# andrewjong/SwapNet

Hardware: NVIDIA H100
Metric: images/sec (G+D fwd+bwd) warp-stage 512x512 (higher is better)
Workload: dtype fp16/bf16-split x3 tensor-core products, fp32 accumulate (fp32-faithful)

## Files before the change

### swapnet_b200/csrc/common.cuh

```cuda
#pragma once
#include <cuda_runtime.h>
#include <cuda.h>
#include <cuda_bf16.h>
#include <cuda_fp16.h>
#include <stdint.h>
#include <stdio.h>
#include <string.h>

void sn_set_error(const char* fmt, ...);
#define SN_OK 0
#define SN_ERR_INVALID (-1)
#define SN_ERR_CUDA (-2)
#define SN_ERR_UNSUPPORTED (-3)
#define SN_NUM_SMS 132
#ifndef SN_FMT_BF16
#define SN_FMT_BF16 0
#define SN_FMT_F16 1
#endif

#define SN_CHECK_CUDA(expr)                                                        \
  do {                                                                             \
    cudaError_t _e = (expr);                                                       \
    if (_e != cudaSuccess) {                                                       \
      sn_set_error("%s:%d CUDA error %s: %s", __FILE__, __LINE__, #expr,           \
                   cudaGetErrorString(_e));                                        \
      return SN_ERR_CUDA;                                                          \
    }                                                                              \
  } while (0)

#define SN_REQUIRE(cond, ...)                                                      \
  do {                                                                             \
    if (!(cond)) {                                                                 \
      sn_set_error(__VA_ARGS__);                                                   \
      return SN_ERR_INVALID;                                                       \
    }                                                                              \
  } while (0)

#ifdef __CUDACC__

__device__ __forceinline__ uint32_t smem_u32(const void* p) {
  return static_cast<uint32_t>(__cvta_generic_to_shared(p));
}

__device__ __forceinline__ bool elect_one_sync() {
  uint32_t pred = 0;
  asm volatile(
      "{\n\t"
      ".reg .pred P;\n\t"
      "elect.sync _|P, 0xffffffff;\n\t"
      "selp.b32 %0, 1, 0, P;\n\t"
      "}\n"
      : "=r"(pred));
  return pred != 0;
}

__device__ __forceinline__ void mbar_init(uint64_t* bar, uint32_t count) {
  asm volatile("mbarrier.init.shared::cta.b64 [%0], %1;" ::"r"(smem_u32(bar)), "r"(count));
}
__device__ __forceinline__ void mbar_fence_init() {
  asm volatile("fence.mbarrier_init.release.cluster;" ::: "memory");
}
__device__ __forceinline__ void mbar_expect_tx(uint64_t* bar, uint32_t bytes) {
  asm volatile("mbarrier.arrive.expect_tx.shared::cta.b64 _, [%0], %1;" ::"r"(smem_u32(bar)),
               "r"(bytes)
               : "memory");
}
__device__ __forceinline__ void mbar_arrive(uint64_t* bar) {
  asm volatile("mbarrier.arrive.shared::cta.b64 _, [%0];" ::"r"(smem_u32(bar)) : "memory");
}
__device__ __forceinline__ bool mbar_try_wait(uint64_t* bar, uint32_t parity) {
  uint32_t ok;
  asm volatile(
      "{\n\t"
      ".reg .pred P;\n\t"
      "mbarrier.try_wait.parity.shared::cta.b64 P, [%1], %2;\n\t"
      "selp.b32 %0, 1, 0, P;\n\t"
      "}\n"
      : "=r"(ok)
      : "r"(smem_u32(bar)), "r"(parity)
      : "memory");
  return ok != 0;
}
__device__ __forceinline__ void mbar_wait(uint64_t* bar, uint32_t parity) {
  uint32_t spins = 0;
  while (!mbar_try_wait(bar, parity)) {
    if (++spins > (1u << 28)) __trap();
  }
}

__device__ __forceinline__ void tma_prefetch_desc(const void* desc) {
  asm volatile("prefetch.tensormap [%0];" ::"l"(reinterpret_cast<uint64_t>(desc)) : "memory");
}
__device__ __forceinline__ void tma_load_2d(const void* desc, uint64_t* bar, void* dst, int c0,
                                            int c1) {
  asm volatile(
      "cp.async.bulk.tensor.2d.shared::cluster.global.mbarrier::complete_tx::bytes"
      " [%0], [%1, {%3, %4}], [%2];"
      :
      : "r"(smem_u32(dst)), "l"(reinterpret_cast<uint64_t>(desc)), "r"(smem_u32(bar)), "r"(c0),
        "r"(c1)
      : "memory");
}
__device__ __forceinline__ void tma_load_3d(const void* desc, uint64_t* bar, void* dst, int c0, int c1, int c2) {
  asm volatile(
      "cp.async.bulk.tensor.3d.shared::cluster.global.mbarrier::complete_tx::bytes"
      " [%0], [%1, {%3, %4, %5}], [%2];"
      :
      : "r"(smem_u32(dst)), "l"(reinterpret_cast<uint64_t>(desc)), "r"(smem_u32(bar)), "r"(c0), "r"(c1), "r"(c2)
      : "memory");
}
__device__ __forceinline__ void tma_load_5d(const void* desc, uint64_t* bar, void* dst, int c0,
                                            int c1, int c2, int c3, int c4) {
  asm volatile(
      "cp.async.bulk.tensor.5d.shared::cluster.global.mbarrier::complete_tx::bytes"
      " [%0], [%1, {%3, %4, %5, %6, %7}], [%2];"
      :
      : "r"(smem_u32(dst)), "l"(reinterpret_cast<uint64_t>(desc)), "r"(smem_u32(bar)), "r"(c0),
        "r"(c1), "r"(c2), "r"(c3), "r"(c4)
      : "memory");
}

__device__ __forceinline__ void wgmma_fence() { asm volatile("wgmma.fence.sync.aligned;" ::: "memory"); }
__device__ __forceinline__ void wgmma_commit() { asm volatile("wgmma.commit_group.sync.aligned;" ::: "memory"); }
template <int N>
__device__ __forceinline__ void wgmma_wait() {
  asm volatile("wgmma.wait_group.sync.aligned %0;" ::"n"(N) : "memory");
}
template <int R>
__device__ __forceinline__ void wgmma_fence_acc(float (&d)[R]) {
#pragma unroll
  for (int i = 0; i < R; ++i) asm volatile("" : "+f"(d[i])::"memory");
}

template <int N, bool F16>
struct Wgmma;
template <> struct Wgmma<16, false> {
  template <int TA, int TB>
  static __device__ __forceinline__ void mma(float (&d)[8], uint64_t a, uint64_t b, int scale_d) {
    asm volatile(
        "{\n.reg .pred p;\nsetp.ne.b32 p, %10, 0;\n"
        "wgmma.mma_async.sync.aligned.m64n16k16.f32.bf16.bf16 "
        "{%0, %1, %2, %3, %4, %5, %6, %7}, %8, %9, p, 1, 1, %11, %12;\n}\n"
        : "+f"(d[0]), "+f"(d[1]), "+f"(d[2]), "+f"(d[3]), "+f"(d[4]), "+f"(d[5]), "+f"(d[6]), "+f"(d[7])
        : "l"(a), "l"(b), "r"(scale_d), "n"(TA), "n"(TB));
  }
};
template <> struct Wgmma<16, true> {
  template <int TA, int TB>
  static __device__ __forceinline__ void mma(float (&d)[8], uint64_t a, uint64_t b, int scale_d) {
    asm volatile(
        "{\n.reg .pred p;\nsetp.ne.b32 p, %10, 0;\n"
        "wgmma.mma_async.sync.aligned.m64n16k16.f32.f16.f16 "
        "{%0, %1, %2, %3, %4, %5, %6, %7}, %8, %9, p, 1, 1, %11, %12;\n}\n"
        : "+f"(d[0]), "+f"(d[1]), "+f"(d[2]), "+f"(d[3]), "+f"(d[4]), "+f"(d[5]), "+f"(d[6]), "+f"(d[7])
        : "l"(a), "l"(b), "r"(scale_d), "n"(TA), "n"(TB));
  }
};
template <> struct Wgmma<32, false> {
// ... 145 lines not shown
```

### swapnet_b200/csrc/gemm_tc.cu

```cuda
#include "common.cuh"
#include "plan.h"

namespace {

constexpr int kBlockM = 128;
constexpr int kTileRing = 4;
constexpr int kTileBytes = 16384;
constexpr int kConsumerWarps = 8;
constexpr int kProducerWarp = kConsumerWarps;
constexpr int kThreads = (kConsumerWarps + 1) * 32;

template <int NSPLIT>
struct Cfg {
  static constexpr int kPlanes = NSPLIT == 3 ? 2 : 1;
  static constexpr int kStages = NSPLIT == 3 ? 3 : 6;
  static constexpr int kStageBytes = kPlanes * 2 * kTileBytes;
  static constexpr int kSmemBytes = kStages * kStageBytes + 1024;
};

__device__ __forceinline__ float apply_act(float v, int act) {
  if (act == SN_ACT_TANH) return tanhf(v);
  return v;
}

__device__ __forceinline__ float quad_col_sum(float v) {
  v += __shfl_xor_sync(0xffffffffu, v, 4);
  v += __shfl_xor_sync(0xffffffffu, v, 8);
  v += __shfl_xor_sync(0xffffffffu, v, 16);
  return v;
}

template <int NSPLIT, int CW, int BN, bool F16>
__global__ void __launch_bounds__(kThreads, 1)
tap_gemm_kernel(const __grid_constant__ TapGemmParams p, const int m_tiles, const int n_tiles, const int total_tiles) {
  const auto tile_coords = [&](int tile, int& mt, int& nt, int& z) {
    nt = tile % n_tiles;
    const int rest = tile / n_tiles;
    mt = rest % m_tiles;
    z = rest / m_tiles;
  };
  using C = Cfg<NSPLIT>;
  extern __shared__ uint8_t smem_raw[];
  __shared__ __align__(8) uint64_t full_bar[C::kStages];
  __shared__ __align__(8) uint64_t empty_bar[C::kStages];
  __shared__ __align__(8) uint64_t tr_full[kTileRing];
  __shared__ __align__(8) uint64_t tr_empty[kTileRing];
  __shared__ int tile_ring[kTileRing];

  const uint32_t smem_base = (smem_u32(smem_raw) + 1023u) & ~1023u;
  uint8_t* smem = smem_raw + (smem_base - smem_u32(smem_raw));
  const int warp = threadIdx.x >> 5;
  const int lane = threadIdx.x & 31;

  constexpr int cw = CW;
  constexpr int tps = 64 / cw;
  const int tpp = p.ntaps / p.nphase;
  const int k_iters = cw == 64 ? tpp * p.chunks : tpp / tps;

  if (threadIdx.x == 0) {
    for (int s = 0; s < C::kStages; ++s) {
      mbar_init(&full_bar[s], 1);
      mbar_init(&empty_bar[s], 2);
    }
    for (int r = 0; r < kTileRing; ++r) {
      mbar_init(&tr_full[r], 1);
      mbar_init(&tr_empty[r], kConsumerWarps);
    }
    mbar_fence_init();
  }
  if (warp == kProducerWarp && lane == 0) {
    for (int pl = 0; pl < C::kPlanes; ++pl) {
      tma_prefetch_desc(&p.tmA[pl]);
      tma_prefetch_desc(&p.tmB[pl]);
    }
  }
  __syncthreads();

  if (warp == kProducerWarp) {
    if (lane == 0) {
      const uint32_t stage_tx = C::kPlanes * (p.a_rows * 128 + p.block_n * 128);
      uint32_t it = 0, tcount = 0;
      for (int tile = blockIdx.x;; ++tcount) {
        const int next = tile < total_tiles ? (int)gridDim.x + atomicAdd(p.tile_counter, 1) : total_tiles;
        const uint32_t slot = tcount % kTileRing, rph = (tcount / kTileRing) & 1;
        mbar_wait(&tr_empty[slot], rph ^ 1);
        tile_ring[slot] = tile < total_tiles ? tile : -1;
        mbar_arrive(&tr_full[slot]);
        if (tile >= total_tiles) break;
        int mt, nt, z;
        tile_coords(tile, mt, nt, z);
        const int ncol0 = nt * p.block_n;
        const int tap0 = z * tpp;
        const int w0 = (mt % p.tiles_w) * p.tw;
// ... 116 lines not shown
        optr[h] = p.out + (long long)gn[h] * p.out_sn + (long long)(gh[h] * p.omh + p.ooh + ph_h) * p.out_sh +
                  (long long)(gw[h] * p.omw + p.oow + ph_w) * p.out_sw + ncol0;
      }
#pragma unroll
      for (int i = 0; i < BN / 8; ++i) {
        const int c = 8 * i + 2 * quad;
        if (BN > 16 && 8 * i >= p.block_n) break;
        if (p.stack_slot) {
#pragma unroll
          for (int h = 0; h < 2; ++h) {
            if (!valid[h]) continue;
#pragma unroll
            for (int e = 0; e < 2; ++e) {
              const int col = ncol0 + c + e;
              const int ph = col / p.stack_slot, ch = col - ph * p.stack_slot;
              if (ph < 4 && ch < p.stack_c) {
                float v = acc[4 * i + 2 * h + e] * oscale;
                if (p.bias) v += p.bias[ch];
                float* o = p.out + (long long)gn[h] * p.out_sn + (long long)(gh[h] * p.omh + (ph >> 1)) * p.out_sh +
                           (long long)(gw[h] * p.omw + (ph & 1)) * p.out_sw + ch;
                *o = apply_act(v, p.act);
              }
            }
          }
        } else if (p.stats) {
          if (ncol0 + 8 * i >= p.n_valid) continue;
          float v[2][2];
#pragma unroll
          for (int h = 0; h < 2; ++h) {
#pragma unroll
            for (int e = 0; e < 2; ++e) {
              float t = acc[4 * i + 2 * h + e] * oscale;
              if (p.bias) t += p.bias[ncol0 + c + e];
              v[h][e] = valid[h] ? t : 0.f;
            }
            if (valid[h]) *reinterpret_cast<float2*>(optr[h] + c) = make_float2(v[h][0], v[h][1]);
          }
          const float s0 = quad_col_sum(v[0][0] + v[1][0]);
          const float s1 = quad_col_sum(v[0][1] + v[1][1]);
          const float q0 = quad_col_sum(v[0][0] * v[0][0] + v[1][0] * v[1][0]);
          const float q1 = quad_col_sum(v[0][1] * v[0][1] + v[1][1] * v[1][1]);
          if (lane < 4) {
            const int tn = (mt / (p.tiles_w * p.tiles_h)) * p.nb;
            double* sp = p.stats + ((long long)tn * p.n_valid + ncol0 + c) * 2;
            atomicAdd(sp, (double)s0);
            atomicAdd(sp + 1, (double)q0);
            atomicAdd(sp + 2, (double)s1);
            atomicAdd(sp + 3, (double)q1);
          }
        } else {
#pragma unroll
          for (int h = 0; h < 2; ++h) {
            if (!valid[h]) continue;
            float v0 = acc[4 * i + 2 * h] * oscale, v1 = acc[4 * i + 2 * h + 1] * oscale;
            const int col = ncol0 + c;
            if (p.vec4 && col + 1 < p.n_valid) {
              if (p.bias) {
                const float2 bb = *reinterpret_cast<const float2*>(p.bias + col);
                v0 += bb.x; v1 += bb.y;
              }
              *reinterpret_cast<float2*>(optr[h] + c) = make_float2(apply_act(v0, p.act), apply_act(v1, p.act));
            } else {
              if (col < p.n_valid) optr[h][c] = apply_act(p.bias ? v0 + p.bias[col] : v0, p.act);
              if (col + 1 < p.n_valid) optr[h][c + 1] = apply_act(p.bias ? v1 + p.bias[col + 1] : v1, p.act);
            }
          }
        }
      }
    }
  }

  __syncthreads();
  if (threadIdx.x == 0) {
    __threadfence();
    if (atomicAdd(p.tile_counter + 1, 1) == (int)gridDim.x - 1) {
      p.tile_counter[0] = 0;
      p.tile_counter[1] = 0;
      __threadfence();
    }
  }
}

template <int NSPLIT, int BN, bool F16, bool DET>
__global__ void __launch_bounds__(kThreads, 1)
wgrad_gemm_kernel(const __grid_constant__ WgradParams p) {
  using C = Cfg<NSPLIT>;
  extern __shared__ uint8_t smem_raw[];
  __shared__ __align__(8) uint64_t full_bar[C::kStages];
  __shared__ __align__(8) uint64_t empty_bar[C::kStages];

  const uint32_t smem_base = (smem_u32(smem_raw) + 1023u) & ~1023u;
  uint8_t* smem = smem_raw + (smem_base - smem_u32(smem_raw));
  const int warp = threadIdx.x >> 5;
  const int lane = threadIdx.x & 31;

  const int m_tile = blockIdx.x / p.n_tiles;
  const int n_tile = blockIdx.x - m_tile * p.n_tiles;
  const bool grouped = p.ngroups > 0;
  const int tap_i = grouped ? p.gstart[blockIdx.y] : blockIdx.y;
  const int gsize = grouped ? p.gsize[blockIdx.y] : 1;
  const int m0 = m_tile * kBlockM;
  const int ncol0 = n_tile * p.block_n;
  const int total = p.tiles_w * p.tiles_h * p.tiles_n;
  const int kt0 = (int)(((long long)total * blockIdx.z) / gridDim.z);
  const int kt1 = (int)(((long long)total * (blockIdx.z + 1)) / gridDim.z);
  const int k_iters = kt1 - kt0;
  const int ycw = p.y_chunk;
  const int y_blocks = ycw == 64 ? p.block_n / 64 : gsize;
  const int y_block_bytes = 64 * ycw * 2;

  if (threadIdx.x == 0) {
    for (int s = 0; s < C::kStages; ++s) {
      mbar_init(&full_bar[s], 1);
      mbar_init(&empty_bar[s], 2);
    }
    mbar_fence_init();
  }
  if (warp == kProducerWarp && lane == 0) {
    for (int pl = 0; pl < C::kPlanes; ++pl) {
      tma_prefetch_desc(&p.tmX[pl]);
      tma_prefetch_desc(&p.tmY[pl]);
    }
  }
  __syncthreads();

  if (k_iters > 0) {
    if (warp == kProducerWarp) {
      if (lane == 0) {
        const TapDesc xt = p.xtaps[tap_i];
        const uint32_t stage_tx = C::kPlanes * (2 * 8192 + y_blocks * y_block_bytes);
        for (int it = 0; it < k_iters; ++it) {
          const int s = it % C::kStages;
          const uint32_t ph = (it / C::kStages) & 1;
          mbar_wait(&empty_bar[s], ph ^ 1);
          mbar_expect_tx(&full_bar[s], stage_tx);
          const int kt = kt0 + it;
          const int tw_i = kt % p.tiles_w;
          const int th_i = (kt / p.tiles_w) % p.tiles_h;
          const int tn_i = kt / (p.tiles_w * p.tiles_h);
          const int w0 = tw_i * p.tw, h0 = th_i * p.th, n0 = tn_i * p.nb;
          uint8_t* st = smem + s * C::kStageBytes;
          if (p.x_merged) {
            for (int b = 0; b < 2; ++b)
              tma_load_5d(&p.tmX[0], &full_bar[s], st + b * 16384, xt.c_off + m0 + b * 64, w0 + xt.dw, h0 + xt.dh,
                          n0, 0);
          } else {
#pragma unroll
            for (int pl = 0; pl < C::kPlanes; ++pl)
              for (int b = 0; b < 2; ++b)
                tma_load_5d(&p.tmX[pl], &full_bar[s], st + pl * kTileBytes + b * 8192,
                            xt.c_off + m0 + b * 64, w0 + xt.dw, xt.hp, h0 + xt.dh, n0);
          }
          if (p.y_merged) {
            const TapDesc yt = p.ytaps[tap_i];
            for (int b = 0; b < y_blocks; ++b)
              tma_load_5d(&p.tmY[0], &full_bar[s], st + C::kPlanes * kTileBytes + b * 16384,
                          yt.c_off + ncol0 + b * 64, w0 + yt.dw, h0 + yt.dh, n0, 0);
          } else {
#pragma unroll
            for (int pl = 0; pl < C::kPlanes; ++pl)
              for (int b = 0; b < y_blocks; ++b) {
                const TapDesc yt = p.ytaps[grouped ? tap_i + b : tap_i];
                tma_load_5d(&p.tmY[pl], &full_bar[s],
                            st + (C::kPlanes + pl) * kTileBytes + b * y_block_bytes,
                            yt.c_off + (grouped ? 0 : ncol0 + b * 64), w0 + yt.dw, yt.hp, h0 + yt.dh, n0);
              }
          }
        }
      }
    } else if (warp < kProducerWarp) {
      const int wg = warp >> 2;
      float acc[BN / 2], part[BN / 2];
#pragma unroll
      for (int i = 0; i < BN / 2; ++i) acc[i] = 0.f;
      const uint32_t y_layout = gmma_layout_of_chunk(ycw);
      const uint32_t y_sbo = 8u * ycw * 2u;
      const uint32_t x_lbo = p.x_merged ? 16384u : 8192u;
      const uint32_t x_lo_off = p.x_merged ? 8192u : (uint32_t)kTileBytes;
      const uint32_t y_lbo = p.y_merged ? 16384u : (uint32_t)y_block_bytes;
      const uint32_t y_lo_off = p.y_merged ? 8192u : (uint32_t)kTileBytes;
      for (int it = 0; it < k_iters; ++it) {
        const int s = it % C::kStages;
        const uint32_t ph = (it / C::kStages) & 1;
        mbar_wait(&full_bar[s], ph);
        const uint32_t st = smem_base + s * C::kStageBytes;
        const uint64_t x_hi = gmma_smem_desc(st + wg * x_lbo, x_lbo, 1024);
        const uint64_t y_hi = gmma_smem_desc(st + C::kPlanes * kTileBytes, y_lbo, y_sbo, y_layout);
        const uint64_t x_lo = gmma_smem_desc(st + x_lo_off + wg * x_lbo, x_lbo, 1024);
        const uint64_t y_lo = gmma_smem_desc(st + C::kPlanes * kTileBytes + y_lo_off, y_lbo, y_sbo, y_layout);
        wgmma_fence();
#pragma unroll
        for (int k = 0; k < 4; ++k) {
          const uint64_t xadv = (uint64_t)(k * 128);
          const uint64_t yadv = (uint64_t)((k * 16 * ycw * 2) >> 4);
          Wgmma<BN, F16>::template mma<1, 1>(part, x_hi + xadv, y_hi + yadv, k != 0);
          if (NSPLIT == 3) {
            Wgmma<BN, F16>::template mma<1, 1>(part, x_lo + xadv, y_hi + yadv, 1);
            Wgmma<BN, F16>::template mma<1, 1>(part, x_hi + xadv, y_lo + yadv, 1);
          }
        }
        wgmma_commit();
        wgmma_wait<0>();
        wgmma_fence_acc(part);
        if ((threadIdx.x & 127) == 0) mbar_arrive(&empty_bar[s]);
#pragma unroll
        for (int i = 0; i < BN / 2; ++i) acc[i] += part[i];
      }
      const int quad = lane & 3;
      const int row0 = m0 + wg * 64 + (warp & 3) * 16 + (lane >> 2);
#pragma unroll
      for (int h = 0; h < 2; ++h) {
        const int row = row0 + 8 * h;
        if (row >= p.rows_valid) continue;
        float* orow = p.out + (long long)row * p.s_row;
        float* wrow = DET ? p.det_ws + (long long)blockIdx.z * p.det_count + (long long)row * p.cols_valid : nullptr;
#pragma unroll
        for (int i = 0; i < BN / 8; ++i) {
#pragma unroll
          for (int e = 0; e < 2; ++e) {
            const int c = 8 * i + 2 * quad + e;
            const float v = acc[4 * i + 2 * h + e];
            if (!grouped) {
              const int col = ncol0 + c;
              if (c < p.block_n && col < p.cols_valid) {
                if constexpr (DET) wrow[(long long)tap_i * p.rows_valid * p.cols_valid + col] = v;
                else atomicAdd(orow + p.tap_off[tap_i] + (long long)col * p.s_col, v);
              }
            } else {
              const int b = c / ycw;
              const int cbase = c - b * ycw;
              if (b < gsize && cbase < p.cols_valid) {
                if constexpr (DET) wrow[(long long)(tap_i + b) * p.rows_valid * p.cols_valid + cbase] = v;
                else atomicAdd(orow + p.tap_off[tap_i + b] + (long long)cbase * p.s_col, v);
              }
            }
          }
        }
      }
    }
  }
}

__global__ void __launch_bounds__(256) wgrad_det_sum_kernel(const __grid_constant__ WgradParams p, int ksplit) {
  const long long rc = (long long)p.rows_valid * p.cols_valid;
  for (long long e = blockIdx.x * (long long)blockDim.x + threadIdx.x; e < p.det_count;
       e += (long long)gridDim.x * blockDim.x) {
    float s = p.det_ws[e];
    for (int z = 1; z < ksplit; ++z) s += p.det_ws[(long long)z * p.det_count + e];
    const int tap = (int)(e / rc);
    const long long r = e - tap * rc;
    const int row = (int)(r / p.cols_valid), col = (int)(r - (long long)row * p.cols_valid);
    p.out[(long long)row * p.s_row + p.tap_off[tap] + (long long)col * p.s_col] += s;
  }
}

}

void sn_count_launch(int n);
typedef CUresult (*PFN_encodeTiled)(CUtensorMap*, CUtensorMapDataType, cuuint32_t, void*,
                                    const cuuint64_t*, const cuuint64_t*, const cuuint32_t*,
                                    const cuuint32_t*, CUtensorMapInterleave, CUtensorMapSwizzle,
                                    CUtensorMapL2promotion, CUtensorMapFloatOOBfill);

static PFN_encodeTiled get_encode_fn() {
  static PFN_encodeTiled fn = nullptr;
  if (!fn) {
    void* ptr = nullptr;
    cudaDriverEntryPointQueryResult qres;
    cudaError_t e = cudaGetDriverEntryPoint("cuTensorMapEncodeTiled", &ptr, cudaEnableDefault, &qres);
    if (e != cudaSuccess || qres != cudaDriverEntryPointSuccess || !ptr) return nullptr;
    fn = reinterpret_cast<PFN_encodeTiled>(ptr);
  }
  return fn;
}

int sn_make_act_map(CUtensorMap* tm, const void* base, int N, int H, int W, int C, int pitch,
                    int parity, int box_w, int box_h, int box_n, int chunk = 64, long long plane_stride = 0) {
  PFN_encodeTiled enc = get_encode_fn();
  SN_REQUIRE(enc != nullptr, "cuTensorMapEncodeTiled driver entry point unavailable");
  SN_REQUIRE(pitch % 8 == 0 && ((uintptr_t)base % 16) == 0,
             "activation plane needs 16-B aligned base and pitch %% 8 == 0 (pitch=%d)", pitch);
  SN_REQUIRE(box_w >= 1 && box_h >= 1 && box_n >= 1 && box_w <= 256 && box_h <= 256 && box_n <= 256,
             "bad TMA box %d x %d x %d", box_w, box_h, box_n);
  cuuint64_t dims[5];
  cuuint64_t strides[4];
  const cuuint64_t e = 2;
  cuuint32_t box[5] = {(cuuint32_t)chunk, (cuuint32_t)box_w, 1, (cuuint32_t)box_h, (cuuint32_t)box_n};
  if (plane_stride > 0) {
    SN_REQUIRE(plane_stride % 16 == 0, "merged planes: 16-B aligned plane stride");
    if (!parity) {
      dims[0] = C; dims[1] = W; dims[2] = H; dims[3] = N; dims[4] = 2;
      strides[0] = (cuuint64_t)pitch * e;
      strides[1] = (cuuint64_t)W * pitch * e;
    } else {
      SN_REQUIRE(H % 2 == 0 && W % 2 == 0, "parity view needs even H, W (got %d x %d)", H, W);
      dims[0] = (cuuint64_t)(W + 1) * pitch + C; dims[1] = W / 2; dims[2] = H / 2; dims[3] = N; dims[4] = 2;
      strides[0] = (cuuint64_t)2 * pitch * e;
      strides[1] = (cuuint64_t)2 * W * pitch * e;
    }
    strides[2] = (cuuint64_t)H * W * pitch * e;
    strides[3] = (cuuint64_t)plane_stride;
    box[2] = (cuuint32_t)box_h; box[3] = (cuuint32_t)box_n; box[4] = 2;
  } else if (!parity) {
    dims[0] = C; dims[1] = W; dims[2] = 1; dims[3] = H; dims[4] = N;
    strides[0] = (cuuint64_t)pitch * e;
    strides[1] = (cuuint64_t)W * pitch * e;
    strides[2] = (cuuint64_t)W * pitch * e;
    strides[3] = (cuuint64_t)H * W * pitch * e;
  } else {
    SN_REQUIRE(H % 2 == 0 && W % 2 == 0, "parity view needs even H, W (got %d x %d)", H, W);
    dims[0] = (cuuint64_t)pitch + C; dims[1] = W / 2; dims[2] = 2; dims[3] = H / 2; dims[4] = N;
    strides[0] = (cuuint64_t)2 * pitch * e;
    strides[1] = (cuuint64_t)W * pitch * e;
    strides[2] = (cuuint64_t)2 * W * pitch * e;
    strides[3] = (cuuint64_t)H * W * pitch * e;
  }
  SN_REQUIRE(chunk == 64 || chunk == 32 || chunk == 16, "row chunk must be 64, 32 or 16 channels (got %d)", chunk);
  cuuint32_t estr[5] = {1, 1, 1, 1, 1};
// ... 277 lines not shown
  for (int t = 0; t < d->ntaps; ++t) {
    p.xtaps[t].c_off = d->xtaps[t].c_off; p.xtaps[t].dw = (short)d->xtaps[t].dw;
    p.xtaps[t].dh = (short)d->xtaps[t].dh; p.xtaps[t].hp = (short)d->xtaps[t].hp;
    p.ytaps[t].c_off = d->ytaps[t].c_off; p.ytaps[t].dw = (short)d->ytaps[t].dw;
    p.ytaps[t].dh = (short)d->ytaps[t].dh; p.ytaps[t].hp = (short)d->ytaps[t].hp;
    p.tap_off[t] = d->tap_off[t];
  }
  p.block_n = d->block_n;
  p.m_tiles = (d->rows_valid + kBlockM - 1) / kBlockM;
  p.n_tiles = y_chunk == 64 ? (d->cols_valid + d->block_n - 1) / d->block_n : 1;
  p.rows_valid = d->rows_valid;
  p.cols_valid = d->cols_valid;
  p.out = d->out;
  p.s_row = d->s_row;
  p.s_col = d->s_col;
  p.x_fmt = d->x_fmt;
  p.y_fmt = d->y_fmt;
  int rc;
  const void* x_pl[2] = {d->x_hi, d->x_lo};
  const void* y_pl[2] = {d->y_hi, d->y_lo};
  {
    const long long x_ps = d->nsplit == 3 ? (const char*)d->x_lo - (const char*)d->x_hi : 0;
    const long long y_ps = d->nsplit == 3 ? (const char*)d->y_lo - (const char*)d->y_hi : 0;
    p.x_merged = x_ps > 0 && x_ps % 16 == 0 && tw * th * nb == 64;
    p.y_merged = y_ps > 0 && y_ps % 16 == 0 && tw * th * nb == 64 && y_chunk == 64 && d->ngroups == 0;
    for (int t = 0; t < d->ntaps; ++t) {
      if (p.x_merged && d->x_parity) p.xtaps[t].c_off += p.xtaps[t].hp * d->x_w * d->x_pitch;
      if (p.y_merged && d->y_parity) p.ytaps[t].c_off += p.ytaps[t].hp * d->y_w * d->y_pitch;
    }
    for (int pl = 0; pl < (d->nsplit == 3 ? 2 : 1); ++pl) {
      if (!(p.x_merged && pl == 1)) {
        rc = sn_make_act_map(&p.tmX[pl], x_pl[pl], d->x_n, d->x_h, d->x_w, d->x_c, d->x_pitch,
                             d->x_parity, tw, th, nb, 64, p.x_merged ? x_ps : 0);
        if (rc) return rc;
      }
      if (!(p.y_merged && pl == 1)) {
        rc = sn_make_act_map(&p.tmY[pl], y_pl[pl], d->y_n, d->y_h, d->y_w, d->y_c, d->y_pitch,
                             d->y_parity, tw, th, nb, y_chunk, p.y_merged ? y_ps : 0);
        if (rc) return rc;
      }
    }
    if (p.x_merged) p.tmX[1] = p.tmX[0];
    if (p.y_merged) p.tmY[1] = p.tmY[0];
  }
  plan->nsplit = d->nsplit;
  const int base_ctas = p.m_tiles * p.n_tiles * grid_y;
  const int total = p.tiles_w * p.tiles_h * p.tiles_n;
  const int ks = wgrad_ksplit(d, base_ctas, total, sm_count);
  plan->grid = dim3(p.m_tiles * p.n_tiles, grid_y, ks);
  p.det_ws = nullptr;
  p.det_count = 0;
  plan->ws_bytes = 0;
  if (d->deterministic) {
    for (int t = 0; t < d->ntaps; ++t)
      for (int u = 0; u < t; ++u)
        SN_REQUIRE(d->tap_off[t] != d->tap_off[u], "deterministic wgrad: taps %d and %d share tap_off", u, t);
    p.det_count = (long long)d->ntaps * d->rows_valid * d->cols_valid;
    plan->ws_bytes = sizeof(float) * (size_t)ks * p.det_count;
    SN_CHECK_CUDA(cudaMalloc(&p.det_ws, plan->ws_bytes));
  }
  return SN_OK;
}

int sn_wgrad_plan_ksplit(const sn_wgrad_desc* d, int sm_count) {
  SN_REQUIRE(d && d->ntaps >= 1 && d->ntaps <= SN_MAX_TAPS, "wgrad_ksplit: bad descriptor");
  int th, tw, nb;
  pick_patch(d->m_h, d->m_w, 64, &th, &tw, &nb);
  const int total = ((d->m_w + tw - 1) / tw) * ((d->m_h + th - 1) / th) * ((d->m_n + nb - 1) / nb);
  const int y_chunk = d->y_chunk ? d->y_chunk : 64;
  const int grid_y = (y_chunk != 64 && d->ngroups > 0) ? d->ngroups : d->ntaps;
  const int m_tiles = (d->rows_valid + kBlockM - 1) / kBlockM;
  const int n_tiles = y_chunk == 64 ? (d->cols_valid + d->block_n - 1) / d->block_n : 1;
  return wgrad_ksplit(d, m_tiles * n_tiles * grid_y, total, sm_count);
}

template <int NSPLIT, int BN, bool F16, bool DET>
static int launch_wgrad_k(const WgradPlan* plan, cudaStream_t stream) {
  static bool attr_done = false;
  if (!attr_done) {
    SN_CHECK_CUDA(cudaFuncSetAttribute(wgrad_gemm_kernel<NSPLIT, BN, F16, DET>,
                                       cudaFuncAttributeMaxDynamicSharedMemorySize, Cfg<NSPLIT>::kSmemBytes));
    attr_done = true;
  }
  wgrad_gemm_kernel<NSPLIT, BN, F16, DET><<<plan->grid, kThreads, Cfg<NSPLIT>::kSmemBytes, stream>>>(plan->p);
  SN_CHECK_CUDA(cudaGetLastError());
  return SN_OK;
}

template <int NSPLIT, int BN, bool F16>
static int launch_wgrad(const WgradPlan* plan, cudaStream_t stream) {
  if (!plan->p.det_ws) return launch_wgrad_k<NSPLIT, BN, F16, false>(plan, stream);
  const int rc = launch_wgrad_k<NSPLIT, BN, F16, true>(plan, stream);
  if (rc) return rc;
  long long g = (plan->p.det_count + 255) / 256;
  if (g > SN_NUM_SMS * 8) g = SN_NUM_SMS * 8;
  wgrad_det_sum_kernel<<<(int)g, 256, 0, stream>>>(plan->p, (int)plan->grid.z);
  SN_CHECK_CUDA(cudaGetLastError());
  sn_count_launch(1);
  return SN_OK;
}

template <int NSPLIT, bool F16>
static int launch_wgrad_n(const WgradPlan* plan, cudaStream_t stream) {
  switch (mma_n(plan->p.block_n)) {
    case 16: return launch_wgrad<NSPLIT, 16, F16>(plan, stream);
    case 32: return launch_wgrad<NSPLIT, 32, F16>(plan, stream);
    case 64: return launch_wgrad<NSPLIT, 64, F16>(plan, stream);
    case 96: return launch_wgrad<NSPLIT, 96, F16>(plan, stream);
    default: return launch_wgrad<NSPLIT, 128, F16>(plan, stream);
  }
}

int sn_wgrad_plan_launch(const WgradPlan* plan, cudaStream_t stream) {
  const bool f16 = plan->p.x_fmt == SN_FMT_F16;
  if (plan->nsplit == 3) return f16 ? launch_wgrad_n<3, true>(plan, stream) : launch_wgrad_n<3, false>(plan, stream);
  return f16 ? launch_wgrad_n<1, true>(plan, stream) : launch_wgrad_n<1, false>(plan, stream);
}
```

Baseline: 139.7.

## Drop wgrad producer warp and overlap consecutive wgmma stages with double-buffered partials

Removes the dedicated TMA producer warp from the wgrad GEMM. Consumer warpgroup leaders now issue refill loads when both groups have released a slot, tracked with a shared release counter. Each stage's wgmma runs asynchronously with ping-pong partial accumulators, retiring the previous stage only after the next is committed, so tensor-core work overlaps with accumulation and barrier handling. The risks are loads being issued from the consumer critical path, which can stall refills, and higher register pressure from the second partial array.

After: 125.0, median of 6. -10.5%, worse.

```diff
diff --git a/swapnet_b200/csrc/common.cuh b/swapnet_b200/csrc/common.cuh
--- a/swapnet_b200/csrc/common.cuh
+++ b/swapnet_b200/csrc/common.cuh
@@ -74,6 +74,19 @@
       "{\n\t"
       ".reg .pred P;\n\t"
       "mbarrier.try_wait.parity.shared::cta.b64 P, [%1], %2;\n\t"
+      "selp.b32 %0, 1, 0, P;\n\t"
+      "}\n"
+      : "=r"(ok)
+      : "r"(smem_u32(bar)), "r"(parity)
+      : "memory");
+  return ok != 0;
+}
+__device__ __forceinline__ bool mbar_test_wait(uint64_t* bar, uint32_t parity) {
+  uint32_t ok;
+  asm volatile(
+      "{\n\t"
+      ".reg .pred P;\n\t"
+      "mbarrier.test_wait.parity.shared::cta.b64 P, [%1], %2;\n\t"
       "selp.b32 %0, 1, 0, P;\n\t"
       "}\n"
       : "=r"(ok)
diff --git a/swapnet_b200/csrc/gemm_tc.cu b/swapnet_b200/csrc/gemm_tc.cu
--- a/swapnet_b200/csrc/gemm_tc.cu
+++ b/swapnet_b200/csrc/gemm_tc.cu
@@ -9,6 +9,7 @@
 constexpr int kConsumerWarps = 8;
 constexpr int kProducerWarp = kConsumerWarps;
 constexpr int kThreads = (kConsumerWarps + 1) * 32;
+constexpr int kWgradThreads = kConsumerWarps * 32;
 
 template <int NSPLIT>
 struct Cfg {
@@ -291,12 +292,13 @@
 }
 
 template <int NSPLIT, int BN, bool F16, bool DET>
-__global__ void __launch_bounds__(kThreads, 1)
+__global__ void __launch_bounds__(kWgradThreads, 1)
 wgrad_gemm_kernel(const __grid_constant__ WgradParams p) {
   using C = Cfg<NSPLIT>;
   extern __shared__ uint8_t smem_raw[];
   __shared__ __align__(8) uint64_t full_bar[C::kStages];
   __shared__ __align__(8) uint64_t empty_bar[C::kStages];
+  __shared__ int slot_releases[C::kStages];
 
   const uint32_t smem_base = (smem_u32(smem_raw) + 1023u) & ~1023u;
   uint8_t* smem = smem_raw + (smem_base - smem_u32(smem_raw));
@@ -322,127 +324,146 @@
     for (int s = 0; s < C::kStages; ++s) {
       mbar_init(&full_bar[s], 1);
       mbar_init(&empty_bar[s], 2);
+      slot_releases[s] = 0;
     }
     mbar_fence_init();
-  }
-  if (warp == kProducerWarp && lane == 0) {
     for (int pl = 0; pl < C::kPlanes; ++pl) {
       tma_prefetch_desc(&p.tmX[pl]);
       tma_prefetch_desc(&p.tmY[pl]);
     }
   }
   __syncthreads();
-
-  if (k_iters > 0) {
-    if (warp == kProducerWarp) {
-      if (lane == 0) {
-        const TapDesc xt = p.xtaps[tap_i];
-        const uint32_t stage_tx = C::kPlanes * (2 * 8192 + y_blocks * y_block_bytes);
-        for (int it = 0; it < k_iters; ++it) {
-          const int s = it % C::kStages;
-          const uint32_t ph = (it / C::kStages) & 1;
-          mbar_wait(&empty_bar[s], ph ^ 1);
-          mbar_expect_tx(&full_bar[s], stage_tx);
-          const int kt = kt0 + it;
-          const int tw_i = kt % p.tiles_w;
-          const int th_i = (kt / p.tiles_w) % p.tiles_h;
-          const int tn_i = kt / (p.tiles_w * p.tiles_h);
-          const int w0 = tw_i * p.tw, h0 = th_i * p.th, n0 = tn_i * p.nb;
-          uint8_t* st = smem + s * C::kStageBytes;
-          if (p.x_merged) {
-            for (int b = 0; b < 2; ++b)
-              tma_load_5d(&p.tmX[0], &full_bar[s], st + b * 16384, xt.c_off + m0 + b * 64, w0 + xt.dw, h0 + xt.dh,
-                          n0, 0);
-          } else {
-#pragma unroll
-            for (int pl = 0; pl < C::kPlanes; ++pl)
-              for (int b = 0; b < 2; ++b)
-                tma_load_5d(&p.tmX[pl], &full_bar[s], st + pl * kTileBytes + b * 8192,
-                            xt.c_off + m0 + b * 64, w0 + xt.dw, xt.hp, h0 + xt.dh, n0);
+  if (k_iters <= 0) return;
+
+  const auto load_stage = [&](int it) {
+    const int s = it % C::kStages;
+    const TapDesc xt = p.xtaps[tap_i];
+    mbar_expect_tx(&full_bar[s], C::kPlanes * (2 * 8192 + y_blocks * y_block_bytes));
+    const int kt = kt0 + it;
+    const int tw_i = kt % p.tiles_w;
+    const int th_i = (kt / p.tiles_w) % p.tiles_h;
+    const int tn_i = kt / (p.tiles_w * p.tiles_h);
+    const int w0 = tw_i * p.tw, h0 = th_i * p.th, n0 = tn_i * p.nb;
+    uint8_t* st = smem + s * C::kStageBytes;
+    if (p.x_merged) {
+      for (int b = 0; b < 2; ++b)
+        tma_load_5d(&p.tmX[0], &full_bar[s], st + b * 16384, xt.c_off + m0 + b * 64, w0 + xt.dw, h0 + xt.dh, n0, 0);
+    } else {
+#pragma unroll
+      for (int pl = 0; pl < C::kPlanes; ++pl)
+        for (int b = 0; b < 2; ++b)
+          tma_load_5d(&p.tmX[pl], &full_bar[s], st + pl * kTileBytes + b * 8192,
+                      xt.c_off + m0 + b * 64, w0 + xt.dw, xt.hp, h0 + xt.dh, n0);
+    }
+    if (p.y_merged) {
+      const TapDesc yt = p.ytaps[tap_i];
+      for (int b = 0; b < y_blocks; ++b)
+        tma_load_5d(&p.tmY[0], &full_bar[s], st + C::kPlanes * kTileBytes + b * 16384,
+                    yt.c_off + ncol0 + b * 64, w0 + yt.dw, h0 + yt.dh, n0, 0);
+    } else {
+#pragma unroll
+      for (int pl = 0; pl < C::kPlanes; ++pl)
+        for (int b = 0; b < y_blocks; ++b) {
+          const TapDesc yt = p.ytaps[grouped ? tap_i + b : tap_i];
+          tma_load_5d(&p.tmY[pl], &full_bar[s],
+                      st + (C::kPlanes + pl) * kTileBytes + b * y_block_bytes,
+                      yt.c_off + (grouped ? 0 : ncol0 + b * 64), w0 + yt.dw, yt.hp, h0 + yt.dh, n0);
+        }
+    }
+  };
+  if (threadIdx.x == 0)
+    for (int it = 0; it < C::kStages && it < k_iters; ++it) load_stage(it);
+  __syncwarp();
+
+  const int wg = warp >> 2;
+  float acc[BN / 2], part0[BN / 2], part1[BN / 2];
+#pragma unroll
+  for (int i = 0; i < BN / 2; ++i) acc[i] = 0.f;
+  const uint32_t y_layout = gmma_layout_of_chunk(ycw);
+  const uint32_t y_sbo = 8u * ycw * 2u;
+  const uint32_t x_lbo = p.x_merged ? 16384u : 8192u;
+  const uint32_t x_lo_off = p.x_merged ? 8192u : (uint32_t)kTileBytes;
+  const uint32_t y_lbo = p.y_merged ? 16384u : (uint32_t)y_block_bytes;
+  const uint32_t y_lo_off = p.y_merged ? 8192u : (uint32_t)kTileBytes;
+  const auto retire = [&](float (&part)[BN / 2], int it) {
+    wgmma_fence_acc(part);
+    if ((threadIdx.x & 127) == 0) {
+      const int s = it % C::kStages;
+      mbar_arrive(&empty_bar[s]);
+      if ((atomicAdd(&slot_releases[s], 1) & 1) && it + C::kStages < k_iters) {
+        mbar_wait(&empty_bar[s], (it / C::kStages) & 1);
+        load_stage(it + C::kStages);
+      }
+    }
+    __syncwarp();
+#pragma unroll
+    for (int i = 0; i < BN / 2; ++i) acc[i] += part[i];
+  };
+  const auto stage = [&](float (&part)[BN / 2], float (&prev)[BN / 2], int it) {
+    const int s = it % C::kStages;
+    const uint32_t ph = (it / C::kStages) & 1;
+    bool prev_pending = it > 0;
+    if (prev_pending && !mbar_test_wait(&full_bar[s], ph)) {
+      wgmma_wait<0>();
+      retire(prev, it - 1);
+      prev_pending = false;
+    }
+    mbar_wait(&full_bar[s], ph);
+    const uint32_t st = smem_base + s * C::kStageBytes;
+    const uint64_t x_hi = gmma_smem_desc(st + wg * x_lbo, x_lbo, 1024);
+    const uint64_t y_hi = gmma_smem_desc(st + C::kPlanes * kTileBytes, y_lbo, y_sbo, y_layout);
+    const uint64_t x_lo = gmma_smem_desc(st + x_lo_off + wg * x_lbo, x_lbo, 1024);
+    const uint64_t y_lo = gmma_smem_desc(st + C::kPlanes * kTileBytes + y_lo_off, y_lbo, y_sbo, y_layout);
+    wgmma_fence();
+#pragma unroll
+    for (int k = 0; k < 4; ++k) {
+      const uint64_t xadv = (uint64_t)(k * 128);
+      const uint64_t yadv = (uint64_t)((k * 16 * ycw * 2) >> 4);
+      Wgmma<BN, F16>::template mma<1, 1>(part, x_hi + xadv, y_hi + yadv, k != 0);
+      if (NSPLIT == 3) {
+        Wgmma<BN, F16>::template mma<1, 1>(part, x_lo + xadv, y_hi + yadv, 1);
+        Wgmma<BN, F16>::template mma<1, 1>(part, x_hi + xadv, y_lo + yadv, 1);
+      }
+    }
+    wgmma_commit();
+    if (prev_pending) {
+      wgmma_wait<1>();
+      retire(prev, it - 1);
+    }
+  };
+  for (int it = 0; it < k_iters; it += 2) {
+    stage(part0, part1, it);
+    if (it + 1 < k_iters) stage(part1, part0, it + 1);
+  }
+  wgmma_wait<0>();
+  if (k_iters & 1) retire(part0, k_iters - 1);
+  else retire(part1, k_iters - 1);
+  const int quad = lane & 3;
+  const int row0 = m0 + wg * 64 + (warp & 3) * 16 + (lane >> 2);
+#pragma unroll
+  for (int h = 0; h < 2; ++h) {
+    const int row = row0 + 8 * h;
+    if (row >= p.rows_valid) continue;
+    float* orow = p.out + (long long)row * p.s_row;
+    float* wrow = DET ? p.det_ws + (long long)blockIdx.z * p.det_count + (long long)row * p.cols_valid : nullptr;
+#pragma unroll
+    for (int i = 0; i < BN / 8; ++i) {
+#pragma unroll
+      for (int e = 0; e < 2; ++e) {
+        const int c = 8 * i + 2 * quad + e;
+        const float v = acc[4 * i + 2 * h + e];
+        if (!grouped) {
+          const int col = ncol0 + c;
+          if (c < p.block_n && col < p.cols_valid) {
+            if constexpr (DET) wrow[(long long)tap_i * p.rows_valid * p.cols_valid + col] = v;
+            else atomicAdd(orow + p.tap_off[tap_i] + (long long)col * p.s_col, v);
           }
-          if (p.y_merged) {
-            const TapDesc yt = p.ytaps[tap_i];
-            for (int b = 0; b < y_blocks; ++b)
-              tma_load_5d(&p.tmY[0], &full_bar[s], st + C::kPlanes * kTileBytes + b * 16384,
-                          yt.c_off + ncol0 + b * 64, w0 + yt.dw, h0 + yt.dh, n0, 0);
-          } else {
-#pragma unroll
-            for (int pl = 0; pl < C::kPlanes; ++pl)
-              for (int b = 0; b < y_blocks; ++b) {
-                const TapDesc yt = p.ytaps[grouped ? tap_i + b : tap_i];
-                tma_load_5d(&p.tmY[pl], &full_bar[s],
-                            st + (C::kPlanes + pl) * kTileBytes + b * y_block_bytes,
-                            yt.c_off + (grouped ? 0 : ncol0 + b * 64), w0 + yt.dw, yt.hp, h0 + yt.dh, n0);
-              }
-          }
-        }
-      }
-    } else if (warp < kProducerWarp) {
-      const int wg = warp >> 2;
-      float acc[BN / 2], part[BN / 2];
-#pragma unroll
-      for (int i = 0; i < BN / 2; ++i) acc[i] = 0.f;
-      const uint32_t y_layout = gmma_layout_of_chunk(ycw);
-      const uint32_t y_sbo = 8u * ycw * 2u;
-      const uint32_t x_lbo = p.x_merged ? 16384u : 8192u;
-      const uint32_t x_lo_off = p.x_merged ? 8192u : (uint32_t)kTileBytes;
-      const uint32_t y_lbo = p.y_merged ? 16384u : (uint32_t)y_block_bytes;
-      const uint32_t y_lo_off = p.y_merged ? 8192u : (uint32_t)kTileBytes;
-      for (int it = 0; it < k_iters; ++it) {
-        const int s = it % C::kStages;
-        const uint32_t ph = (it / C::kStages) & 1;
-        mbar_wait(&full_bar[s], ph);
-        const uint32_t st = smem_base + s * C::kStageBytes;
-        const uint64_t x_hi = gmma_smem_desc(st + wg * x_lbo, x_lbo, 1024);
-        const uint64_t y_hi = gmma_smem_desc(st + C::kPlanes * kTileBytes, y_lbo, y_sbo, y_layout);
-        const uint64_t x_lo = gmma_smem_desc(st + x_lo_off + wg * x_lbo, x_lbo, 1024);
-        const uint64_t y_lo = gmma_smem_desc(st + C::kPlanes * kTileBytes + y_lo_off, y_lbo, y_sbo, y_layout);
-        wgmma_fence();
-#pragma unroll
-        for (int k = 0; k < 4; ++k) {
-          const uint64_t xadv = (uint64_t)(k * 128);
-          const uint64_t yadv = (uint64_t)((k * 16 * ycw * 2) >> 4);
-          Wgmma<BN, F16>::template mma<1, 1>(part, x_hi + xadv, y_hi + yadv, k != 0);
-          if (NSPLIT == 3) {
-            Wgmma<BN, F16>::template mma<1, 1>(part, x_lo + xadv, y_hi + yadv, 1);
-            Wgmma<BN, F16>::template mma<1, 1>(part, x_hi + xadv, y_lo + yadv, 1);
-          }
-        }
-        wgmma_commit();
-        wgmma_wait<0>();
-        wgmma_fence_acc(part);
-        if ((threadIdx.x & 127) == 0) mbar_arrive(&empty_bar[s]);
-#pragma unroll
-        for (int i = 0; i < BN / 2; ++i) acc[i] += part[i];
-      }
-      const int quad = lane & 3;
-      const int row0 = m0 + wg * 64 + (warp & 3) * 16 + (lane >> 2);
-#pragma unroll
-      for (int h = 0; h < 2; ++h) {
-        const int row = row0 + 8 * h;
-        if (row >= p.rows_valid) continue;
-        float* orow = p.out + (long long)row * p.s_row;
-        float* wrow = DET ? p.det_ws + (long long)blockIdx.z * p.det_count + (long long)row * p.cols_valid : nullptr;
-#pragma unroll
-        for (int i = 0; i < BN / 8; ++i) {
-#pragma unroll
-          for (int e = 0; e < 2; ++e) {
-            const int c = 8 * i + 2 * quad + e;
-            const float v = acc[4 * i + 2 * h + e];
-            if (!grouped) {
-              const int col = ncol0 + c;
-              if (c < p.block_n && col < p.cols_valid) {
-                if constexpr (DET) wrow[(long long)tap_i * p.rows_valid * p.cols_valid + col] = v;
-                else atomicAdd(orow + p.tap_off[tap_i] + (long long)col * p.s_col, v);
-              }
-            } else {
-              const int b = c / ycw;
-              const int cbase = c - b * ycw;
-              if (b < gsize && cbase < p.cols_valid) {
-                if constexpr (DET) wrow[(long long)(tap_i + b) * p.rows_valid * p.cols_valid + cbase] = v;
-                else atomicAdd(orow + p.tap_off[tap_i + b] + (long long)cbase * p.s_col, v);
-              }
-            }
+        } else {
+          const int b = c / ycw;
+          const int cbase = c - b * ycw;
+          if (b < gsize && cbase < p.cols_valid) {
+            if constexpr (DET) wrow[(long long)(tap_i + b) * p.rows_valid * p.cols_valid + cbase] = v;
+            else atomicAdd(orow + p.tap_off[tap_i + b] + (long long)cbase * p.s_col, v);
           }
         }
       }
@@ -886,7 +907,7 @@
                                        cudaFuncAttributeMaxDynamicSharedMemorySize, Cfg<NSPLIT>::kSmemBytes));
     attr_done = true;
   }
-  wgrad_gemm_kernel<NSPLIT, BN, F16, DET><<<plan->grid, kThreads, Cfg<NSPLIT>::kSmemBytes, stream>>>(plan->p);
+  wgrad_gemm_kernel<NSPLIT, BN, F16, DET><<<plan->grid, kWgradThreads, Cfg<NSPLIT>::kSmemBytes, stream>>>(plan->p);
   SN_CHECK_CUDA(cudaGetLastError());
   return SN_OK;
 }
```
